# hustvl/InfiniteVL

Measured on AMD Instinct MI355X. Metric: prefill tok/s + decode tok/s, InfiniteVL-3B @128K seq, higher is better.
Workload: dtype bf16; 1 GPU; InfiniteVL-3B (36 layers: 9 SWA + 27 Gated DeltaNet, random-init bf16) streaming prefill, 256-token hipGraph chunk steps, SWA window 4096 (full); global_batch=1, seq_len=150016, parallelism=dp1 (batch-sharded replicas, one logits all-gather)

## Files before the change

### include/ivl_hip.h

```cpp
#ifndef IVL_HIP_H
#define IVL_HIP_H

#include <stddef.h>
#include <stdint.h>

#ifdef __cplusplus
extern "C" {
#endif

#define IVL_ABI_VERSION 11

#define IVL_API __attribute__((visibility("default")))

#define IVL_BF16 0
#define IVL_F32 2
#define IVL_FP8_E4M3 3

#define IVL_OK 0
#define IVL_ERR_INVALID_ARG (-1)
#define IVL_ERR_UNSUPPORTED (-2)
#define IVL_ERR_WORKSPACE (-3)
#define IVL_ERR_LAUNCH (-4)
#define IVL_ERR_SYNC (-5)

IVL_API int ivl_abi_version(void);
IVL_API const char* ivl_last_error(void);

IVL_API int ivl_gdn_recurrent_fwd(const void* q, const void* k, const void* v, const float* g, const void* beta,
                          void* o, const void* h0, int h0_dtype, void* ht, int ht_dtype,
                          int B, int T, int H, int K, int V, float scale, int use_qk_l2norm, void* stream);
IVL_API int ivl_gdn_recurrent_f16_fwd(const void* q, const void* k, const void* v, const float* g, const void* beta,
                              void* o, const void* h0, int h0_dtype, void* ht, int ht_dtype,
                              int B, int T, int H, int K, int V, float scale, int use_qk_l2norm, void* stream);

IVL_API size_t ivl_gdn_chunk_workspace_bytes(int B, int T, int H, int K, int V);
IVL_API int ivl_gdn_chunk_fwd(const void* q, const void* k, const void* v, const float* g, const void* beta,
                      void* o, const void* h0, int h0_dtype, void* ht, int ht_dtype,
                      int B, int T, int H, int K, int V, float scale, int use_qk_l2norm, int mma_dtype,
                      void* workspace, size_t workspace_bytes, void* stream);

#define IVL_GDN_SYNC_BYTES 16384
IVL_API int ivl_gdn_chunk_fused_fwd(const void* proj, int64_t ld, int col_q, int col_k, int col_v, int col_a, int col_b,
                            const void* wq, const void* wk, const void* wv, const void* sq_in, const void* sk_in,
                            const void* sv_in, void* sq_out, void* sk_out, void* sv_out, const float* A_log,
                            const float* dt_bias, void* o, const void* h0, int h0_dtype, void* ht, int ht_dtype, int B,
                            int T, int H, int K, int V, int conv_width, float scale, int mma_dtype, void* workspace,
                            size_t workspace_bytes, void* sync, void* stream);
IVL_API int ivl_gdn_sync_status(const void* sync, void* stream);
IVL_API int ivl_gdn_sync_reset(void* sync, void* stream);
#define IVL_GDN_RESIDENT_QUERY (-2147483647 - 1)
IVL_API int ivl_gdn_resident_blocks(int override_blocks);

IVL_API int ivl_gdn_gate_fwd(const void* a, const void* b, const float* A_log, const float* dt_bias,
                     float* g, void* beta, int rows, int H, void* stream);

IVL_API int ivl_short_conv_fwd(const void* x, const void* weight, const void* state_in, void* y, void* state_out,
                       int B, int T, int D, int W, int apply_silu, void* stream);
IVL_API int ivl_short_conv_bias_fwd(const void* x, const void* weight, const void* bias, const void* state_in, void* y, void* state_out,
                            int B, int T, int D, int W, int apply_silu, void* stream);

IVL_API int ivl_rmsnorm_swish_gate_fwd(const void* x, const void* gate, const void* weight, void* y,
                               int rows, int N, float eps, void* stream);
IVL_API int ivl_rmsnorm_swish_gate_res_fwd(const void* x, const void* gate, const void* weight, const void* residual, int residual_dtype,
                                   void* residual_out, int residual_out_dtype, void* y, int rows, int N, float eps, void* stream);

IVL_API int ivl_mrope_fwd(void* q, void* k, const void* cos, const void* sin,
                  int B, int T, int Hq, int Hkv, int d, int s0, int s1, int s2, void* stream);

typedef struct ivl_swa_args {
  const void* q;
  const void* k_new;
  const void* v_new;
  const void* k_cache;
  const void* v_cache;
  void* o;
  int64_t q_sb, q_st, q_sh;
  int64_t kn_sb, kn_st, kn_sh;
  int B, T, T_new, Hq, Hkv, d;
  int cache_capacity;
  int window;
  int64_t pos;
  const int64_t* pos_dev;
  float scaling;
  void* workspace;
  size_t workspace_bytes;
  const void* rope_cos;
  const void* rope_sin;
  int rope_s0, rope_s1;
  int mma_dtype;
  int append_new;
  int64_t pos_min;
} ivl_swa_args;

IVL_API size_t ivl_swa_workspace_bytes(int B, int T, int Hq, int d);
IVL_API size_t ivl_swa_ring256_workspace_bytes(int B, int T, int Hq, int Hkv, int d, int cache_capacity);
IVL_API int ivl_swa_fwd(const ivl_swa_args* args, void* stream);
IVL_API int ivl_swa_decode_rows_fwd(const ivl_swa_args* args, const int64_t* pos_rows, void* stream);

IVL_API int ivl_swa_cache_append(const void* k_new, const void* v_new, int64_t kn_sb, int64_t kn_st, int64_t kn_sh,
                         void* k_cache, void* v_cache, int B, int T, int Hkv, int d, int cache_capacity,
                         int64_t pos, const int64_t* pos_dev, const void* rope_cos, const void* rope_sin,
                         int rope_s0, int rope_s1, void* stream);

IVL_API int ivl_rope_tables_fwd(const int64_t* position_ids, const float* inv_freq, void* cos_out, void* sin_out, int rows,
                        int half_dim, float attention_scaling, void* stream);

IVL_API size_t ivl_vision_attn_workspace_bytes(int S, int H, int d, int max_seqlen);
IVL_API int ivl_vision_attn_fwd(const void* q, const void* k, const void* v, void* o,
                        int64_t q_st, int64_t q_sh, int64_t k_st, int64_t k_sh, int64_t v_st, int64_t v_sh,
                        int64_t o_st, int64_t o_sh, const int32_t* cu_seqlens, int n_seg, int max_seqlen,
                        int S, int H, int d, float scaling, const float* rope_cos, const float* rope_sin,
                        void* workspace, size_t workspace_bytes, void* stream);

IVL_API int ivl_counter_add(int64_t* counter, int64_t delta, void* stream);


IVL_API int ivl_gdn_prologue_fwd(const void* proj, int64_t ld, int col_q, int col_k, int col_v, int col_a, int col_b,
                         const void* w_q, const void* w_k, const void* w_v,
                         const void* sq_in, const void* sk_in, const void* sv_in,
                         void* sq_out, void* sk_out, void* sv_out,
                         const float* A_log, const float* dt_bias,
                         void* q, void* k, void* v, float* g, void* beta,
                         int B, int T, int H, int Dq, int Dk, int Dv, int W, int apply_silu, void* stream);

IVL_API int ivl_rmsnorm_swish_gate_strided_fwd(const void* x, const void* gate, int64_t gate_ld, int H,
                                       const void* weight, void* y, int rows, int N, float eps, void* stream);

IVL_API int ivl_mrope_strided_fwd(void* q, void* k, int64_t q_ld, int64_t k_ld, const void* cos, const void* sin,
                          int B, int T, int Hq, int Hkv, int d, int s0, int s1, int s2, void* stream);

IVL_API int ivl_add_rmsnorm_fwd(const void* x, const void* residual, const void* weight, void* y, void* h_out,
                        int rows, int N, float eps, void* stream);

IVL_API int ivl_silu_mul_fwd(const void* gate_up, void* y, int64_t rows, int I, void* stream);

IVL_API int ivl_gdn_decode_step_fwd(const void* proj, int64_t ld, int col_q, int col_k, int col_v, int col_g, int col_a,
                            int col_b, const void* conv_wq, const void* conv_wk, const void* conv_wv,
                            void* conv_state_q, void* conv_state_k, void* conv_state_v, const float* A_log,
                            const float* dt_bias, const void* norm_weight, float eps, void* state, int state_dtype,
                            void* y, int B, int H, int K, int V, float scale, void* stream);

IVL_API int ivl_gdn_decode_split_fwd(const void* proj, int64_t ld, int col_q, int col_k, int col_v, int col_a, int col_b,
                             const void* conv_wq, const void* conv_wk, const void* conv_wv, const void* conv_state_q,
                             const void* conv_state_k, void* conv_state_v, const float* A_log, const float* dt_bias,
                             void* state, int state_dtype, void* o_raw, int B, int H, int K, int V, float scale, void* stream);
IVL_API int ivl_gdn_out_linear_small_m_fwd(const void* o_raw, const void* gate, int64_t gate_ld, const void* norm_weight, float eps,
                                   int H, const void* proj, int64_t proj_ld, int col_q, int col_k, void* conv_state_q,
                                   void* conv_state_k, const void* w, const void* bias, void* y, int M, int N, int K, void* stream);

IVL_API int ivl_linear_small_m_fwd(const void* x, const void* w, const void* bias, void* y, int M, int N, int K, void* stream);

IVL_API int ivl_linear_swiglu_small_m_fwd(const void* x, const void* w_gate_up, const void* bias, void* y, int M, int I, int K,
                                  void* stream);

IVL_API int ivl_norm_linear_small_m_fwd(const void* x, const void* residual, const void* norm_weight, float eps, void* h_out,
                                const void* w, const void* bias, void* y, int M, int N, int K, int glu, void* stream);

#ifdef __cplusplus
}
#endif
#endif
```

### infinitevl_amd/_lib.py

```python
from __future__ import annotations

import ctypes
import os
from ctypes import POINTER, Structure, c_char_p, c_float, c_int, c_int64, c_size_t, c_void_p

_HERE = os.path.dirname(os.path.abspath(__file__))
LIB_PATH = os.path.join(_HERE, "libivl_hip.so")

IVL_BF16, IVL_F32, IVL_FP8_E4M3 = 0, 2, 3
IVL_OK = 0
IVL_GDN_SYNC_BYTES = 16384
IVL_GDN_RESIDENT_QUERY = -2147483648
IVL_ERR_INVALID_ARG, IVL_ERR_UNSUPPORTED, IVL_ERR_WORKSPACE, IVL_ERR_LAUNCH, IVL_ERR_SYNC = -1, -2, -3, -4, -5

EXPORTED_SYMBOLS = (
    "ivl_abi_version", "ivl_last_error",
    "ivl_gdn_recurrent_fwd", "ivl_gdn_chunk_workspace_bytes", "ivl_gdn_chunk_fwd", "ivl_gdn_gate_fwd",
    "ivl_short_conv_fwd", "ivl_rmsnorm_swish_gate_fwd", "ivl_mrope_fwd",
    "ivl_swa_workspace_bytes", "ivl_swa_fwd", "ivl_swa_cache_append", "ivl_counter_add",
    "ivl_gdn_prologue_fwd", "ivl_rmsnorm_swish_gate_strided_fwd", "ivl_mrope_strided_fwd",
    "ivl_add_rmsnorm_fwd", "ivl_silu_mul_fwd", "ivl_linear_small_m_fwd",
    "ivl_linear_swiglu_small_m_fwd", "ivl_gdn_decode_step_fwd", "ivl_gdn_chunk_fused_fwd", "ivl_rope_tables_fwd",
    "ivl_vision_attn_workspace_bytes", "ivl_vision_attn_fwd", "ivl_norm_linear_small_m_fwd",
    "ivl_gdn_sync_status", "ivl_gdn_sync_reset", "ivl_gdn_resident_blocks",
    "ivl_short_conv_bias_fwd", "ivl_rmsnorm_swish_gate_res_fwd", "ivl_gdn_recurrent_f16_fwd",
    "ivl_gdn_decode_split_fwd", "ivl_gdn_out_linear_small_m_fwd", "ivl_swa_ring256_workspace_bytes",
    "ivl_swa_decode_rows_fwd",
)


class SwaArgs(Structure):
    _fields_ = [
        ("q", c_void_p), ("k_new", c_void_p), ("v_new", c_void_p), ("k_cache", c_void_p), ("v_cache", c_void_p),
        ("o", c_void_p),
        ("q_sb", c_int64), ("q_st", c_int64), ("q_sh", c_int64),
        ("kn_sb", c_int64), ("kn_st", c_int64), ("kn_sh", c_int64),
        ("B", c_int), ("T", c_int), ("T_new", c_int), ("Hq", c_int), ("Hkv", c_int), ("d", c_int),
        ("cache_capacity", c_int), ("window", c_int),
        ("pos", c_int64), ("pos_dev", c_void_p),
        ("scaling", c_float),
        ("workspace", c_void_p), ("workspace_bytes", c_size_t),
        ("rope_cos", c_void_p), ("rope_sin", c_void_p), ("rope_s0", c_int), ("rope_s1", c_int),
        ("mma_dtype", c_int), ("append_new", c_int),
        ("pos_min", c_int64),
    ]


class IvlError(RuntimeError):
    def __init__(self, code: int, msg: str):
        super().__init__(f"libivl_hip error {code}: {msg}")
        self.code = code


_lib = None


def load(path: str = None) -> ctypes.CDLL:
    global _lib
    if _lib is not None:
        return _lib
    if path is not None:
        globals()["LIB_PATH"] = path
    if not os.path.exists(LIB_PATH):
        raise ImportError(
            f"{LIB_PATH} not found. The MI355X kernels are mandatory (there is no CPU or PyTorch fallback): "
            "build them with `python -c 'import __graft_entry__ as g; g.build()'` or `make -C infinitevl_amd/csrc`.")
    lib = ctypes.CDLL(LIB_PATH)
    vp, i, f, sz, i64 = c_void_p, c_int, c_float, c_size_t, c_int64
    lib.ivl_abi_version.restype = i
    lib.ivl_abi_version.argtypes = []
    lib.ivl_last_error.restype = c_char_p
    lib.ivl_last_error.argtypes = []
    lib.ivl_gdn_recurrent_fwd.restype = i
    lib.ivl_gdn_recurrent_fwd.argtypes = [vp, vp, vp, vp, vp, vp, vp, i, vp, i, i, i, i, i, i, f, i, vp]
    lib.ivl_gdn_chunk_workspace_bytes.restype = sz
    lib.ivl_gdn_chunk_workspace_bytes.argtypes = [i, i, i, i, i]
    lib.ivl_gdn_chunk_fwd.restype = i
    lib.ivl_gdn_chunk_fwd.argtypes = [vp, vp, vp, vp, vp, vp, vp, i, vp, i, i, i, i, i, i, f, i, i, vp, sz, vp]
    lib.ivl_gdn_chunk_fused_fwd.restype = i
    lib.ivl_gdn_chunk_fused_fwd.argtypes = ([vp, c_int64, i, i, i, i, i] + [vp] * 9 + [vp, vp, vp, vp, i, vp, i] +
                                            [i, i, i, i, i, i, f, i, vp, sz, vp, vp])
    if path is None or hasattr(lib, "ivl_gdn_sync_status"):
        lib.ivl_gdn_sync_status.restype = i
        lib.ivl_gdn_sync_status.argtypes = [vp, vp]
        lib.ivl_gdn_sync_reset.restype = i
        lib.ivl_gdn_sync_reset.argtypes = [vp, vp]
        lib.ivl_gdn_resident_blocks.restype = i
        lib.ivl_gdn_resident_blocks.argtypes = [i]
        lib.ivl_short_conv_bias_fwd.restype = i
        lib.ivl_short_conv_bias_fwd.argtypes = [vp, vp, vp, vp, vp, vp, i, i, i, i, i, vp]
        lib.ivl_rmsnorm_swish_gate_res_fwd.restype = i
        lib.ivl_rmsnorm_swish_gate_res_fwd.argtypes = [vp, vp, vp, vp, i, vp, i, vp, i, i, f, vp]
        lib.ivl_gdn_recurrent_f16_fwd.restype = i
        lib.ivl_gdn_recurrent_f16_fwd.argtypes = [vp, vp, vp, vp, vp, vp, vp, i, vp, i, i, i, i, i, i, f, i, vp]
    lib.ivl_rope_tables_fwd.restype = i
    lib.ivl_rope_tables_fwd.argtypes = [vp, vp, vp, vp, i, i, f, vp]
    lib.ivl_vision_attn_workspace_bytes.restype = sz
    lib.ivl_vision_attn_workspace_bytes.argtypes = [i, i, i, i]
    lib.ivl_vision_attn_fwd.restype = i
    lib.ivl_vision_attn_fwd.argtypes = [vp, vp, vp, vp] + [c_int64] * 8 + [vp, i, i, i, i, i, f, vp, vp, vp, sz, vp]
    lib.ivl_gdn_gate_fwd.restype = i
    lib.ivl_gdn_gate_fwd.argtypes = [vp, vp, vp, vp, vp, vp, i, i, vp]
    lib.ivl_short_conv_fwd.restype = i
    lib.ivl_short_conv_fwd.argtypes = [vp, vp, vp, vp, vp, i, i, i, i, i, vp]
    lib.ivl_rmsnorm_swish_gate_fwd.restype = i
    lib.ivl_rmsnorm_swish_gate_fwd.argtypes = [vp, vp, vp, vp, i, i, f, vp]
    lib.ivl_mrope_fwd.restype = i
    lib.ivl_mrope_fwd.argtypes = [vp, vp, vp, vp, i, i, i, i, i, i, i, i, vp]
    lib.ivl_swa_workspace_bytes.restype = sz
    lib.ivl_swa_workspace_bytes.argtypes = [i, i, i, i]
    lib.ivl_swa_ring256_workspace_bytes.restype = sz
    lib.ivl_swa_ring256_workspace_bytes.argtypes = [i, i, i, i, i, i]
    lib.ivl_swa_fwd.restype = i
    lib.ivl_swa_fwd.argtypes = [POINTER(SwaArgs), vp]
    if path is None or hasattr(lib, "ivl_swa_decode_rows_fwd"):
        lib.ivl_swa_decode_rows_fwd.restype = i
        lib.ivl_swa_decode_rows_fwd.argtypes = [POINTER(SwaArgs), vp, vp]
    lib.ivl_swa_cache_append.restype = i
    lib.ivl_swa_cache_append.argtypes = [vp, vp, i64, i64, i64, vp, vp, i, i, i, i, i, i64, vp, vp, vp, i, i, vp]
    lib.ivl_counter_add.restype = i
    lib.ivl_counter_add.argtypes = [vp, i64, vp]
    lib.ivl_gdn_prologue_fwd.restype = i
    lib.ivl_gdn_prologue_fwd.argtypes = [vp, i64, i, i, i, i, i, vp, vp, vp, vp, vp, vp, vp, vp, vp, vp, vp,
                                         vp, vp, vp, vp, vp, i, i, i, i, i, i, i, i, vp]
    lib.ivl_rmsnorm_swish_gate_strided_fwd.restype = i
    lib.ivl_rmsnorm_swish_gate_strided_fwd.argtypes = [vp, vp, i64, i, vp, vp, i, i, f, vp]
    lib.ivl_mrope_strided_fwd.restype = i
    lib.ivl_mrope_strided_fwd.argtypes = [vp, vp, i64, i64, vp, vp, i, i, i, i, i, i, i, i, vp]
    lib.ivl_add_rmsnorm_fwd.restype = i
    lib.ivl_add_rmsnorm_fwd.argtypes = [vp, vp, vp, vp, vp, i, i, f, vp]
    lib.ivl_silu_mul_fwd.restype = i
    lib.ivl_silu_mul_fwd.argtypes = [vp, vp, i64, i, vp]
    lib.ivl_linear_small_m_fwd.restype = i
    lib.ivl_linear_small_m_fwd.argtypes = [vp, vp, vp, vp, i, i, i, vp]
    lib.ivl_gdn_decode_step_fwd.restype = i
    lib.ivl_gdn_decode_step_fwd.argtypes = [vp, i64, i, i, i, i, i, i, vp, vp, vp, vp, vp, vp, vp, vp, vp, f, vp, i,
                                            vp, i, i, i, i, f, vp]
    if path is None or hasattr(lib, "ivl_gdn_decode_split_fwd"):
        lib.ivl_gdn_decode_split_fwd.restype = i
        lib.ivl_gdn_decode_split_fwd.argtypes = [vp, i64, i, i, i, i, i, vp, vp, vp, vp, vp, vp, vp, vp, vp, i, vp, i, i, i, i, f, vp]
        lib.ivl_gdn_out_linear_small_m_fwd.restype = i
        lib.ivl_gdn_out_linear_small_m_fwd.argtypes = [vp, vp, i64, vp, f, i, vp, i64, i, i, vp, vp, vp, vp, vp, i, i, i, vp]
    lib.ivl_linear_swiglu_small_m_fwd.restype = i
    lib.ivl_linear_swiglu_small_m_fwd.argtypes = [vp, vp, vp, vp, i, i, i, vp]
    lib.ivl_norm_linear_small_m_fwd.restype = i
    lib.ivl_norm_linear_small_m_fwd.argtypes = [vp, vp, vp, f, vp, vp, vp, vp, i, i, i, i, vp]
    _lib = lib
    env = os.environ.get("IVL_GDN_RESIDENT_BLOCKS", "")
    if env.strip() and hasattr(lib, "ivl_gdn_resident_blocks"):
        lib.ivl_gdn_resident_blocks(int(env))
    return lib


def check(rc: int) -> None:
    if rc == IVL_OK:
        return
    msg = load().ivl_last_error().decode("utf-8", "replace")
    if rc in (IVL_ERR_INVALID_ARG, IVL_ERR_UNSUPPORTED):
        raise ValueError(f"libivl_hip ({rc}): {msg}")
    raise IvlError(rc, msg)
```

### infinitevl_amd/ops.py

```python
from __future__ import annotations

import contextlib
import ctypes
import os
import threading
import weakref
from typing import Dict, Optional, Tuple

import torch
import torch.nn as nn

from . import _lib
from ._lib import IVL_BF16, IVL_F32, IVL_FP8_E4M3, SwaArgs

_DT_CODE = {torch.bfloat16: IVL_BF16, torch.float32: IVL_F32}
_MMA_CODE = {None: IVL_BF16, "bf16": IVL_BF16, torch.bfloat16: IVL_BF16, "fp8": IVL_FP8_E4M3, "fp8_e4m3": IVL_FP8_E4M3,
             getattr(torch, "float8_e4m3fn", "fp8_e4m3"): IVL_FP8_E4M3}


def mma_code(mma_dtype) -> int:
    try:
        return _MMA_CODE[mma_dtype]
    except KeyError:
        raise ValueError(f"mma_dtype must be None, 'bf16' or 'fp8_e4m3' (got {mma_dtype!r})") from None
# ... 439 lines not shown
        return self.hidden_size * self.kernel_size[0]

    def forward(self, x: torch.Tensor, mask: Optional[torch.Tensor] = None, cache: Optional[torch.Tensor] = None,
                output_final_state: bool = False, cu_seqlens: Optional[torch.Tensor] = None, **kwargs):
        _need_gpu(x)
        if cu_seqlens is not None:
            if x.shape[0] != 1:
                raise ValueError(f"The batch size is expected to be 1 rather than {x.shape[0]} when using `cu_seqlens`.")
            if mask is not None:
                raise ValueError("`mask` and `cu_seqlens` cannot be provided at the same time")
            segs = _varlen_segments(cu_seqlens, x.shape[1])
            if x.dtype != torch.bfloat16:
                raise ValueError(f"ShortConvolution kernel is built for bf16, got {x.dtype}")
            x = x.contiguous()
            D, W = x.shape[2], self.kernel_size[0]
            if cache is not None and (cache.dtype != torch.bfloat16 or not cache.is_contiguous()
                                      or tuple(cache.shape) != (len(segs), D, W)):
                raise ValueError(f"conv cache must be a contiguous bf16 [N,D,W] = {(len(segs), D, W)} tensor (one row block per "
                                 f"sequence of cu_seqlens); got {cache.dtype} {tuple(cache.shape)}")
            state_in = cache
            if cache is None and output_final_state:
                cache = torch.zeros(len(segs), D, W, dtype=x.dtype, device=x.device)
            y = torch.empty_like(x)
            for i, (a, b_) in enumerate(segs):
                if b_ > a:
                    self._launch(x[:, a:b_], y[:, a:b_], None if state_in is None else state_in[i:i + 1],
                                 None if cache is None else cache[i:i + 1], 1, b_ - a, D, W)
            return y, cache
        if mask is not None:
            x = x.mul(mask.unsqueeze(-1))
        if x.dtype != torch.bfloat16:
            raise ValueError(f"ShortConvolution kernel is built for bf16, got {x.dtype}")
        B, T, D = x.shape
        W = self.kernel_size[0]
        x = x.contiguous()
        state_in = cache
        if output_final_state and cache is None:
            cache = torch.empty(B, D, W, dtype=x.dtype, device=x.device)
        if cache is not None and (cache.dtype != torch.bfloat16 or not cache.is_contiguous()
                                  or tuple(cache.shape) != (B, D, W)):
            raise ValueError("conv cache must be a contiguous bf16 [N,D,W] tensor")
        y = torch.empty_like(x)
        self._launch(x, y, state_in, cache, B, T, D, W)
        return y, cache

    def _launch(self, x, y, state_in, state_out, B, T, D, W) -> None:
        w = self.weight
        if w.dtype != torch.bfloat16:
            w = w.to(torch.bfloat16)
        if self.bias is not None:
            _lib.check(_lib.load().ivl_short_conv_bias_fwd(
                _p(x), _p(w.contiguous()), _p(self.bias.to(torch.bfloat16).contiguous()), _p(state_in), _p(y), _p(state_out), B, T, D, W,
                int(self.activation is not None), _stream(x)))
        else:
            _lib.check(_lib.load().ivl_short_conv_fwd(
                _p(x), _p(w.contiguous()), _p(state_in), _p(y), _p(state_out), B, T, D, W,
                int(self.activation is not None), _stream(x)))

    def step(self, x: torch.Tensor, cache: torch.Tensor):
        return self.forward(x, cache=cache, output_final_state=True)


class FusedRMSNormGated(nn.Module):

    def __init__(self, hidden_size: int, elementwise_affine: bool = True, eps: float = 1e-5,
                 activation: str = "swish", device=None, dtype=None):
        super().__init__()
        if activation not in ("swish", "silu"):
            raise ValueError(f"Unsupported activation: {activation}")
        self.hidden_size, self.elementwise_affine, self.eps, self.activation = hidden_size, elementwise_affine, eps, activation
        if elementwise_affine:
            self.weight = nn.Parameter(torch.ones(hidden_size, device=device, dtype=dtype))
        else:
            self.register_parameter("weight", None)
        self.register_parameter("bias", None)

    def forward(self, x: torch.Tensor, g: torch.Tensor, residual=None, prenorm=False, residual_in_fp32=False):
        _need_gpu(x, g, residual)
        if x.dtype != torch.bfloat16:
            raise ValueError(f"FusedRMSNormGated kernel is built for bf16, got {x.dtype}")
        N = x.shape[-1]
        x, g = x.contiguous(), g.contiguous()
        y = torch.empty_like(x)
        if self.weight is None:
            w = torch.ones(N, dtype=torch.bfloat16, device=x.device)
        else:
            w = self.weight if self.weight.dtype == torch.bfloat16 else self.weight.to(torch.bfloat16)
        if residual is not None or prenorm or residual_in_fp32:
            if residual is not None:
                if residual.dtype not in _DT_CODE or tuple(residual.shape) != tuple(x.shape):
                    raise ValueError("residual must be a bf16 / fp32 tensor of x's shape")
                residual = residual.contiguous()
            res_dt = residual.dtype if residual is not None else (torch.float32 if residual_in_fp32 else None)
            res_out = torch.empty(x.shape, dtype=res_dt, device=x.device) if res_dt is not None and (residual is not None or res_dt != x.dtype) else None
            _lib.check(_lib.load().ivl_rmsnorm_swish_gate_res_fwd(
                _p(x), _p(g), _p(w.contiguous()), _p(residual), _DT_CODE[residual.dtype] if residual is not None else IVL_BF16,
                _p(res_out), _DT_CODE[res_out.dtype] if res_out is not None else IVL_BF16, _p(y), x.numel() // N, N, float(self.eps), _stream(x)))
            return y if not prenorm else (y, res_out if res_out is not None else x)
        _lib.check(_lib.load().ivl_rmsnorm_swish_gate_fwd(_p(x), _p(g), _p(w.contiguous()), _p(y),
                                                          x.numel() // N, N, float(self.eps), _stream(x)))
        return y


class RMSNorm(nn.Module):

    def __init__(self, hidden_size: int, elementwise_affine: bool = True, bias: bool = False, eps: float = 1e-5,
                 device=None, dtype=None):
        super().__init__()
        if bias:
            raise NotImplementedError("InfiniteVL's norms carry no bias")
        self.hidden_size, self.elementwise_affine, self.eps = hidden_size, elementwise_affine, eps
        self.register_parameter("weight", None)
        self.register_parameter("bias", None)
        if elementwise_affine:
            self.weight = nn.Parameter(torch.ones(hidden_size, device=device, dtype=dtype))

    def extra_repr(self) -> str:
        return f"{self.hidden_size}, eps={self.eps}" + ("" if self.elementwise_affine else ", elementwise_affine=False")

    def forward(self, x: torch.Tensor, residual=None, prenorm: bool = False, residual_in_fp32: bool = False):
        if residual is not None or prenorm:
            raise NotImplementedError("residual/prenorm are not used by InfiniteVL (std:1341)")
        w = self.weight if self.weight is not None else torch.ones(self.hidden_size, dtype=x.dtype, device=x.device)
        if self.hidden_size == 256 and x.dtype == torch.bfloat16:
            _need_gpu(x)
            xc = x.contiguous()
            y = torch.empty_like(xc)
            _lib.check(_lib.load().ivl_rmsnorm_swish_gate_fwd(_p(xc), None, _p(w.to(torch.bfloat16).contiguous()), _p(y),
                                                              xc.numel() // 256, 256, float(self.eps), _stream(xc)))
            return y
        y, _ = add_rmsnorm(x, None, w, self.eps)
        return y


def get_unpad_data(attention_mask: torch.Tensor):
    lens = attention_mask.sum(dim=-1, dtype=torch.int32)
    indices = torch.nonzero(attention_mask.flatten(), as_tuple=False).flatten()
    cu = torch.nn.functional.pad(torch.cumsum(lens, dim=0, dtype=torch.int32), (1, 0))
    return indices, cu, int(lens.max().item()) if lens.numel() else 0


def index_first_axis(x: torch.Tensor, indices: torch.Tensor) -> torch.Tensor:
    return x.index_select(0, indices)


def pad_input(x: torch.Tensor, indices: torch.Tensor, batch: int, seqlen: int) -> torch.Tensor:
    out = torch.zeros(batch * seqlen, *x.shape[1:], dtype=x.dtype, device=x.device)
    out.index_copy_(0, indices, x)
    return out.view(batch, seqlen, *x.shape[1:])


def gdn_prologue(proj: torch.Tensor, cols, conv_weights, conv_states_in, conv_states_out, A_log32, dt_bias32,
                 H: int, Dq: int, Dk: int, Dv: int):
    _need_gpu(proj)
    B, T, ld = proj.shape
    assert proj.is_contiguous() and proj.dtype == torch.bfloat16
    dev = proj.device
    q = torch.empty(B, T, Dq, dtype=torch.bfloat16, device=dev)
    k = torch.empty(B, T, Dk, dtype=torch.bfloat16, device=dev)
    v = torch.empty(B, T, Dv, dtype=torch.bfloat16, device=dev)
    g = torch.empty(B, T, H, dtype=torch.float32, device=dev)
    beta = torch.empty(B, T, H, dtype=torch.bfloat16, device=dev)
    wq, wk, wv = conv_weights
    si, so = conv_states_in, conv_states_out
    _lib.check(_lib.load().ivl_gdn_prologue_fwd(
        _p(proj), ld, cols[0], cols[1], cols[2], cols[3], cols[4], _p(wq), _p(wk), _p(wv),
        _p(si[0]), _p(si[1]), _p(si[2]), _p(so[0]), _p(so[1]), _p(so[2]), _p(A_log32), _p(dt_bias32),
        _p(q), _p(k), _p(v), _p(g), _p(beta), B, T, H, Dq, Dk, Dv, wq.shape[-1], 1, _stream(proj)))
    return q, k, v, g, beta


def gdn_decode_step(proj: torch.Tensor, cols, conv_weights, conv_states, A_log32, dt_bias32, norm_weight, eps: float,
                    state: torch.Tensor, H: int, K: int, V: int, scale: float) -> torch.Tensor:
    _need_gpu(proj, state)
    B, T, ld = proj.shape
    assert T == 1 and proj.is_contiguous() and proj.dtype == torch.bfloat16 and state.is_contiguous()
    y = torch.empty(B, 1, H * V, dtype=torch.bfloat16, device=proj.device)
    wq, wk, wv = conv_weights
    sq, sk, sv = conv_states
    _lib.check(_lib.load().ivl_gdn_decode_step_fwd(
        _p(proj), ld, cols[0], cols[1], cols[2], cols[3], cols[4], cols[5], _p(wq), _p(wk), _p(wv), _p(sq), _p(sk), _p(sv),
        _p(A_log32), _p(dt_bias32), _p(norm_weight), float(eps), _p(state), _DT_CODE[state.dtype], _p(y), B, H, K, V,
        float(scale), _stream(proj)))
    return y


_SPLIT_DECODE = False


def gdn_decode_split(proj: torch.Tensor, cols, conv_weights, conv_states, A_log32, dt_bias32, state: torch.Tensor,
                     H: int, K: int, V: int, scale: float) -> torch.Tensor:
    _need_gpu(proj, state)
    B, T, ld = proj.shape
    assert T == 1 and proj.is_contiguous() and proj.dtype == torch.bfloat16 and state.is_contiguous()
    o_raw = torch.empty(B, 1, H * V, dtype=torch.bfloat16, device=proj.device)
    wq, wk, wv = conv_weights
    sq, sk, sv = conv_states
    _lib.check(_lib.load().ivl_gdn_decode_split_fwd(
        _p(proj), ld, cols[0], cols[1], cols[2], cols[3], cols[4], _p(wq), _p(wk), _p(wv), _p(sq), _p(sk), _p(sv),
        _p(A_log32), _p(dt_bias32), _p(state), _DT_CODE[state.dtype], _p(o_raw), B, H, K, V, float(scale), _stream(proj)))
    return o_raw


def gdn_out_linear(o_raw: torch.Tensor, proj: torch.Tensor, col_g: int, col_q: int, col_k: int, norm_weight: torch.Tensor, eps: float,
                   conv_state_q: torch.Tensor, conv_state_k: torch.Tensor, weight: torch.Tensor, bias: Optional[torch.Tensor],
                   H: int) -> torch.Tensor:
    _need_gpu(o_raw, proj, weight)
    B, T, ld = proj.shape
    K = o_raw.shape[-1]
    N = weight.shape[0]
    assert T == 1 and o_raw.is_contiguous() and weight.is_contiguous() and weight.dtype == torch.bfloat16
    y = torch.empty(B, 1, N, dtype=torch.bfloat16, device=o_raw.device)
    gate = proj.view(B, ld)[:, col_g:]
    _lib.check(_lib.load().ivl_gdn_out_linear_small_m_fwd(
        _p(o_raw), ctypes.c_void_p(gate.data_ptr()), ld, _p(norm_weight), float(eps), H, _p(proj), ld, col_q, col_k,
        _p(conv_state_q), _p(conv_state_k), _p(weight), _p(bias) if bias is not None else None, _p(y), B, N, K, _stream(o_raw)))
    return y


def rmsnorm_swish_gate_strided(x: torch.Tensor, gate_base: torch.Tensor, gate_ld: int, weight: torch.Tensor,
                               eps: float) -> torch.Tensor:
    _need_gpu(x, gate_base)
    B, T, H, N = x.shape
    y = torch.empty_like(x)
    _lib.check(_lib.load().ivl_rmsnorm_swish_gate_strided_fwd(_p(x), _p(gate_base), gate_ld, H, _p(weight), _p(y),
                                                              B * T * H, N, float(eps), _stream(x)))
    return y


def add_rmsnorm(x: torch.Tensor, residual: Optional[torch.Tensor], weight: torch.Tensor, eps: float):
    _need_gpu(x, residual)
    if x.dtype != torch.bfloat16:
        raise ValueError("add_rmsnorm is built for bf16")
    N = x.shape[-1]
    x = x.contiguous()
    y = torch.empty_like(x)
    h = torch.empty_like(x) if residual is not None else None
    w = weight if weight.dtype == torch.bfloat16 else weight.to(torch.bfloat16)
    _lib.check(_lib.load().ivl_add_rmsnorm_fwd(_p(x), _p(residual.contiguous()) if residual is not None else None,
                                               _p(w), _p(y), _p(h), x.numel() // N, N, float(eps), _stream(x)))
    return y, (h if h is not None else x)


_PRENORM = True


class PreNorm:

    def __init__(self, x: torch.Tensor, residual: Optional[torch.Tensor], weight: torch.Tensor, eps: float):
        self.x = x if x.is_contiguous() else x.contiguous()
        self.residual = None if residual is None else (residual if residual.is_contiguous() else residual.contiguous())
        self.weight = weight if weight.dtype == torch.bfloat16 else weight.to(torch.bfloat16)
        self.eps = float(eps)
        self.h = torch.empty_like(self.x) if residual is not None else self.x
        self.shape, self.dtype, self.device, self.is_cuda = self.x.shape, self.x.dtype, self.x.device, self.x.is_cuda
        self._y = None
        self.done = False

    def size(self, *a):
        return self.x.size(*a)

    def dim(self):
        return self.x.dim()

    def numel(self):
        return self.x.numel()

    def materialize(self) -> torch.Tensor:
        if self._y is None:
            N = self.x.shape[-1]
            self._y = torch.empty_like(self.x)
            _lib.check(_lib.load().ivl_add_rmsnorm_fwd(_p(self.x), _p(self.residual), _p(self.weight), _p(self._y),
                                                       _p(self.h) if self.residual is not None else None,
                                                       self.x.numel() // N, N, self.eps, _stream(self.x)))
            self.done = True
        return self._y


def _prenorm_linear(pn: "PreNorm", weight: torch.Tensor, bias: Optional[torch.Tensor], glu: bool) -> Optional[torch.Tensor]:
    K = weight.shape[-1]
    rows = pn.numel() // K if K else 0
    if not (pn.is_cuda and 1 <= rows <= 4 and pn.dtype == torch.bfloat16 and weight.dtype == torch.bfloat16 and weight.dim() == 2
            and weight.is_contiguous() and K % 8 == 0 and 512 <= K <= 4096 and pn.shape[-1] == K and pn._y is None
            and (bias is None or (bias.dtype == torch.bfloat16 and bias.is_contiguous()))):
        return None
    N = weight.shape[0] // 2 if glu else weight.shape[0]
    y = torch.empty(*pn.shape[:-1], N, dtype=torch.bfloat16, device=pn.device)
    _lib.check(_lib.load().ivl_norm_linear_small_m_fwd(
        _p(pn.x), _p(pn.residual), _p(pn.weight), pn.eps, _p(pn.h) if pn.residual is not None else None,
        _p(weight), _p(bias) if bias is not None else None, _p(y), rows, N, K, 1 if glu else 0, _stream(pn.x)))
    pn.done = True
    return y


def silu_mul(gate_up: torch.Tensor) -> torch.Tensor:
    _need_gpu(gate_up)
    assert gate_up.is_contiguous() and gate_up.dtype == torch.bfloat16
    I = gate_up.shape[-1] // 2
    y = torch.empty(*gate_up.shape[:-1], I, dtype=torch.bfloat16, device=gate_up.device)
    _lib.check(_lib.load().ivl_silu_mul_fwd(_p(gate_up), _p(y), gate_up.numel() // (2 * I), I, _stream(gate_up)))
    return y


def linear(x: torch.Tensor, weight: torch.Tensor, bias: Optional[torch.Tensor] = None) -> torch.Tensor:
    if isinstance(x, PreNorm):
        y = _prenorm_linear(x, weight, bias, False)
        if y is not None:
            return y
        x = x.materialize()
    K = weight.shape[-1]
    rows = x.numel() // K if K else 0
    if (x.is_cuda and 1 <= rows <= 4 and x.dtype == torch.bfloat16 and weight.dtype == torch.bfloat16
            and weight.dim() == 2 and weight.is_contiguous() and K % 8 == 0
            and (bias is None or (bias.dtype == torch.bfloat16 and bias.is_contiguous()))):
        xc = x if x.is_contiguous() else x.contiguous()
        N = weight.shape[0]
        y = torch.empty(*x.shape[:-1], N, dtype=torch.bfloat16, device=x.device)
        _lib.check(_lib.load().ivl_linear_small_m_fwd(_p(xc), _p(weight), _p(bias) if bias is not None else None,
                                                      _p(y), rows, N, K, _stream(x)))
        return y
    return torch.nn.functional.linear(x, weight, bias)


def linear_swiglu(x: torch.Tensor, w_gate_up: torch.Tensor) -> torch.Tensor:
    if isinstance(x, PreNorm):
        y = _prenorm_linear(x, w_gate_up, None, True)
        if y is not None:
            return y
        x = x.materialize()
    K = w_gate_up.shape[-1]
    I = w_gate_up.shape[0] // 2
    rows = x.numel() // K
    if (x.is_cuda and 1 <= rows <= 4 and x.dtype == torch.bfloat16 and w_gate_up.dtype == torch.bfloat16
            and w_gate_up.is_contiguous() and K % 8 == 0):
        xc = x if x.is_contiguous() else x.contiguous()
        y = torch.empty(*x.shape[:-1], I, dtype=torch.bfloat16, device=x.device)
        _lib.check(_lib.load().ivl_linear_swiglu_small_m_fwd(_p(xc), _p(w_gate_up), None, _p(y), rows, I, K, _stream(x)))
        return y
    return silu_mul(linear(x, w_gate_up))


def apply_mrope_strided_inplace(q: torch.Tensor, k: torch.Tensor, cos: torch.Tensor, sin: torch.Tensor, mrope_section):
    _need_gpu(q, k, cos, sin)
    B, T, Hq, d = q.shape
    Hkv = k.shape[2]
    assert q.stride(3) == 1 and q.stride(2) == d and k.stride(3) == 1 and k.stride(2) == d

    def row_stride(t_):
        if T > 1 and B > 1:
            assert t_.stride(0) == T * t_.stride(1), "q/k must be row-uniform views of a [B*T, ld] buffer"
        return t_.stride(1) if T > 1 else t_.stride(0)
    cos = cos.to(torch.bfloat16).contiguous()
    sin = sin.to(torch.bfloat16).contiguous()
    s0, s1, s2 = (int(s) for s in mrope_section)
    _lib.check(_lib.load().ivl_mrope_strided_fwd(_p(q), _p(k), row_stride(q), row_stride(k), _p(cos), _p(sin),
                                                 B, T, Hq, Hkv, d, s0, s1, s2, _stream(q)))
    return q, k


def apply_mrope_inplace(q: torch.Tensor, k: torch.Tensor, cos: torch.Tensor, sin: torch.Tensor, mrope_section):
    _need_gpu(q, k, cos, sin)
    B, T, Hq, d = q.shape
    Hkv = k.shape[2]
    assert q.is_contiguous() and k.is_contiguous() and q.dtype == k.dtype == torch.bfloat16
    cos = cos.to(torch.bfloat16).contiguous()
    sin = sin.to(torch.bfloat16).contiguous()
    if cos.shape[0] != 3 or tuple(cos.shape[1:]) != (B, T, d):
        raise ValueError(f"cos/sin must be [3,B,T,d]; got {tuple(cos.shape)}")
    s0, s1, s2 = (int(s) for s in mrope_section)
    _lib.check(_lib.load().ivl_mrope_fwd(_p(q), _p(k), _p(cos), _p(sin), B, T, Hq, Hkv, d, s0, s1, s2, _stream(q)))
    return q, k


SWA_RING256 = os.environ.get("IVL_SWA_RING256", "1") != "0"
SWA_RING256_CALLS = 0


def swa_forward(
    q: torch.Tensor, k_new: torch.Tensor, v_new: torch.Tensor, *, window: Optional[int], scaling: float,
    k_cache: Optional[torch.Tensor] = None, v_cache: Optional[torch.Tensor] = None,
    pos: int = 0, pos_dev: Optional[torch.Tensor] = None, n_query: Optional[int] = None,
    layout: str = "bthd", mma_dtype=None, rope=None, append: bool = False, pos_min: int = 0, pos_min_holds_in_graph: bool = False,
    pos_rows: Optional[torch.Tensor] = None,
) -> torch.Tensor:
    _need_gpu(q, k_new, v_new, k_cache, v_cache, pos_dev, pos_rows)
    if q.dtype != torch.bfloat16 or k_new.dtype != torch.bfloat16 or v_new.dtype != torch.bfloat16:
        raise ValueError("swa_forward is built for bf16")
    if layout == "bhtd":
        q, k_new, v_new = q.transpose(1, 2), k_new.transpose(1, 2), v_new.transpose(1, 2)
    B, T, Hq, d = q.shape
    T_new, Hkv = k_new.shape[1], k_new.shape[2]
    if n_query is not None:
        assert n_query == T
    if pos_rows is not None:
        if pos_dev is not None or pos != 0 or pos_min != 0:
            raise ValueError("swa_forward: pos_rows excludes pos / pos_dev / pos_min")
        if pos_rows.dtype != torch.int64 or tuple(pos_rows.shape) != (B,) or not pos_rows.is_contiguous():
            raise ValueError(f"swa_forward: pos_rows must be a contiguous int64 [B] = [{B}] tensor; got {pos_rows.dtype} "
                             f"{tuple(pos_rows.shape)}")
        if k_cache is None:
            raise ValueError("swa_forward: pos_rows needs a ring cache (k_cache / v_cache)")
        if T_new != T or T * (Hq // Hkv) > 64:
            raise ValueError(f"swa_forward: pos_rows serves packed decode steps only: T_new == T and T * Hq/Hkv <= 64 "
                             f"(got T={T}, T_new={T_new}, Hq/Hkv={Hq // Hkv})")
        if mma_code(mma_dtype) != IVL_BF16:
            raise ValueError("swa_forward: pos_rows runs in bf16 only (no fp8 decode step)")
    if q.stride(-1) != 1:
        q = q.contiguous()
    if k_new.stride(-1) != 1 or v_new.stride() != k_new.stride():
        k_new, v_new = k_new.contiguous(), v_new.contiguous()
    C = 0
    if k_cache is not None:
        assert k_cache.is_contiguous() and v_cache.is_contiguous() and k_cache.dtype == torch.bfloat16
        assert tuple(k_cache.shape[:2]) == (B, Hkv) and k_cache.shape[3] == d
        C = k_cache.shape[2]
    o = torch.empty(B, T, Hq, d, dtype=torch.bfloat16, device=q.device)
    lib = _lib.load()
    nbytes = lib.ivl_swa_workspace_bytes(B, T, Hq, d)
    pos_min = int(pos_min) if pos_dev is not None else int(pos)
    if pos_rows is not None or not (SWA_RING256 and C > 0 and pos_min >= C and T >= 256 and T_new == T and window == C + 1) or (
            torch.cuda.is_current_stream_capturing() and not pos_min_holds_in_graph):
        pos_min = 0
    else:
        n256 = lib.ivl_swa_ring256_workspace_bytes(B, T, Hq, Hkv, d, C)
        if n256 > 0 and mma_code(mma_dtype) == IVL_BF16:
            global SWA_RING256_CALLS
            SWA_RING256_CALLS += 1
        nbytes = max(nbytes, n256)
    ws = get_workspace(nbytes, q.device, "swa")
    a = SwaArgs()
    a.q, a.k_new, a.v_new, a.k_cache, a.v_cache, a.o = (q.data_ptr(), k_new.data_ptr(), v_new.data_ptr(),
                                                         k_cache.data_ptr() if C else None,
                                                         v_cache.data_ptr() if C else None, o.data_ptr())
    a.q_sb, a.q_st, a.q_sh = q.stride(0), q.stride(1), q.stride(2)
    a.kn_sb, a.kn_st, a.kn_sh = k_new.stride(0), k_new.stride(1), k_new.stride(2)
    a.B, a.T, a.T_new, a.Hq, a.Hkv, a.d = B, T, T_new, Hq, Hkv, d
    a.cache_capacity = C
    a.window = int(window) if window is not None else 0
    a.pos = int(pos)
    a.pos_dev = pos_dev.data_ptr() if pos_dev is not None else None
    a.scaling = float(scaling)
    a.workspace, a.workspace_bytes = ws.data_ptr(), ws.numel()
    a.mma_dtype = mma_code(mma_dtype)
    a.append_new = int(bool(append) and C > 0)
    a.pos_min = pos_min
    if rope is not None:
        cos, sin, sec = _rope_args(rope, B, T, d)
        a.rope_cos, a.rope_sin, a.rope_s0, a.rope_s1 = cos.data_ptr(), sin.data_ptr(), int(sec[0]), int(sec[1])
    if pos_rows is not None:
        _lib.check(lib.ivl_swa_decode_rows_fwd(ctypes.byref(a), pos_rows.data_ptr(), _stream(q)))
    else:
        _lib.check(lib.ivl_swa_fwd(ctypes.byref(a), _stream(q)))
    return o


def _rope_args(rope, B: int, T: int, d: int):
    cos, sin, sec = rope
    if cos.dtype != torch.bfloat16 or not cos.is_contiguous():
        cos = cos.to(torch.bfloat16).contiguous()
    if sin.dtype != torch.bfloat16 or not sin.is_contiguous():
        sin = sin.to(torch.bfloat16).contiguous()
    if tuple(cos.shape) != (3, B, T, d) or tuple(sin.shape) != (3, B, T, d):
        raise ValueError(f"rope cos/sin must be [3,B,T,d] = {(3, B, T, d)}; got {tuple(cos.shape)}")
    return cos, sin, sec


def swa_cache_append(k_new: torch.Tensor, v_new: torch.Tensor, k_cache: torch.Tensor, v_cache: torch.Tensor,
                     pos: int = 0, pos_dev: Optional[torch.Tensor] = None, rope=None) -> None:
    _need_gpu(k_new, v_new, k_cache, v_cache)
    B, T, Hkv, d = k_new.shape
    if k_new.stride(-1) != 1 or v_new.stride() != k_new.stride():
        k_new, v_new = k_new.contiguous(), v_new.contiguous()
    rc = rs = None
    s0 = s1 = 0
    if rope is not None:
        rc, rs, sec = _rope_args(rope, B, T, d)
        s0, s1 = int(sec[0]), int(sec[1])
    _lib.check(_lib.load().ivl_swa_cache_append(
        _p(k_new), _p(v_new), k_new.stride(0), k_new.stride(1), k_new.stride(2), _p(k_cache), _p(v_cache),
        B, T, Hkv, d, k_cache.shape[2], int(pos), _p(pos_dev), _p(rc), _p(rs), s0, s1, _stream(k_new)))


def counter_add(counter: torch.Tensor, delta: int) -> None:
    _lib.check(_lib.load().ivl_counter_add(_p(counter), int(delta), _stream(counter)))


def swa_attention_interface(module, query, key, value, attention_mask=None, dropout: float = 0.0,
                            scaling: Optional[float] = None, sliding_window: Optional[int] = None,
                            position_ids=None, **kwargs):
    if dropout:
        raise NotImplementedError("attention dropout is a training feature; the hot path is inference")
    if scaling is None:
        scaling = query.shape[-1] ** -0.5
    out = swa_forward(query, key, value, window=sliding_window, scaling=scaling, layout="bhtd")
    return out, None
```

Before: 48640 tok/s.

## Add fused 256-row SwiGLU GEMM kernel for prefill chunk MLP

Adds a custom HIP MFMA GEMM specialised for exactly 256 rows that loads x and weight tiles straight into LDS through a 3-stage ring and applies bias plus SiLU-gate times up in the epilogue. In the MLP of the 256-token chunk steps it replaces the hipBLAS linear followed by a separate silu_mul kernel, which removes the round trip of the 2I-wide intermediate through memory. Weight loads use non-temporal hints. The trade-off is that a hand-written kernel may reach lower GEMM throughput than the vendor library.

```diff
diff --git a/include/ivl_hip.h b/include/ivl_hip.h
--- a/include/ivl_hip.h
+++ b/include/ivl_hip.h
@@ -156,6 +156,8 @@
 IVL_API int ivl_norm_linear_small_m_fwd(const void* x, const void* residual, const void* norm_weight, float eps, void* h_out,
                                 const void* w, const void* bias, void* y, int M, int N, int K, int glu, void* stream);
 
+IVL_API int ivl_linear_m256_fwd(const void* x, const void* w, const void* bias, void* y, int M, int N, int K, int glu, void* stream);
+
 #ifdef __cplusplus
 }
 #endif
diff --git a/infinitevl_amd/_lib.py b/infinitevl_amd/_lib.py
--- a/infinitevl_amd/_lib.py
+++ b/infinitevl_amd/_lib.py
@@ -25,7 +25,7 @@
     "ivl_gdn_sync_status", "ivl_gdn_sync_reset", "ivl_gdn_resident_blocks",
     "ivl_short_conv_bias_fwd", "ivl_rmsnorm_swish_gate_res_fwd", "ivl_gdn_recurrent_f16_fwd",
     "ivl_gdn_decode_split_fwd", "ivl_gdn_out_linear_small_m_fwd", "ivl_swa_ring256_workspace_bytes",
-    "ivl_swa_decode_rows_fwd",
+    "ivl_swa_decode_rows_fwd", "ivl_linear_m256_fwd",
 )
 
 
@@ -145,6 +145,8 @@
     lib.ivl_linear_swiglu_small_m_fwd.argtypes = [vp, vp, vp, vp, i, i, i, vp]
     lib.ivl_norm_linear_small_m_fwd.restype = i
     lib.ivl_norm_linear_small_m_fwd.argtypes = [vp, vp, vp, f, vp, vp, vp, vp, i, i, i, i, vp]
+    lib.ivl_linear_m256_fwd.restype = i
+    lib.ivl_linear_m256_fwd.argtypes = [vp, vp, vp, vp, i, i, i, i, vp]
     _lib = lib
     env = os.environ.get("IVL_GDN_RESIDENT_BLOCKS", "")
     if env.strip() and hasattr(lib, "ivl_gdn_resident_blocks"):
diff --git a/infinitevl_amd/csrc/linear_m256.hip b/infinitevl_amd/csrc/linear_m256.hip
--- /dev/null
+++ b/infinitevl_amd/csrc/linear_m256.hip
@@ -0,0 +1,215 @@
+#include "ivl_common.h"
+
+namespace ivl {
+
+constexpr int L256_ROWS = 256;
+constexpr int L256_BK = 64;
+constexpr int L256_KMAX = 16384;
+#ifndef L256_WG_ROWS
+#define L256_WG_ROWS 256
+#endif
+#ifndef L256_STAGES
+#define L256_STAGES 3
+#endif
+#ifndef L256_W_NT
+#define L256_W_NT 1
+#endif
+
+template <bool GLU, int ROWS, int NST>
+struct L256Cfg {
+  static constexpr int NCOL = GLU ? 48 : 64;
+  static constexpr int NW = GLU ? 2 * NCOL : NCOL;
+  static constexpr int NT = NW / 16;
+  static constexpr int WAVES = ROWS / 32;
+  static constexpr int PIECES = (ROWS + NW) / 8;
+  static constexpr int PW_MAX = (PIECES + WAVES - 1) / WAVES;
+  static constexpr int STAGE = (ROWS + NW) * 128;
+  static constexpr int LDS = NST * STAGE;
+};
+
+template <int N>
+__device__ __forceinline__ void l256_vmcnt() {
+  static_assert(N >= 0 && N < 64, "vmcnt immediate");
+  asm volatile("s_waitcnt vmcnt(%0)" ::"n"(N) : "memory");
+}
+
+template <int PW>
+__device__ __forceinline__ void l256_wait_tiles(int ahead) {
+  if (ahead <= 0) l256_vmcnt<0>();
+  else if (ahead == 1) l256_vmcnt<PW>();
+  else l256_vmcnt<2 * PW>();
+}
+
+__device__ __forceinline__ const bf16_t* l256_uniform(const bf16_t* p) {
+  const unsigned long long v = (unsigned long long)p;
+  const unsigned int lo = __builtin_amdgcn_readfirstlane((unsigned int)v), hi = __builtin_amdgcn_readfirstlane((unsigned int)(v >> 32));
+  return (const bf16_t*)(((unsigned long long)hi << 32) | lo);
+}
+
+template <bool GLU, int ROWS, int NST, bool WNT>
+__global__ __launch_bounds__(ROWS * 2) void linear_m256_kernel(const bf16_t* __restrict__ x, const bf16_t* __restrict__ w,
+                                                               const bf16_t* __restrict__ bias, bf16_t* __restrict__ y, int M, int N, int K) {
+  using C = L256Cfg<GLU, ROWS, NST>;
+  static_assert(NST >= 2 && NST <= 3, "ring of 2 or 3 stages");
+  constexpr int AHEAD = NST - 1;
+  extern __shared__ __attribute__((aligned(16))) unsigned char smem[];
+  const int tid = threadIdx.x, lane = tid & 63, wave = __builtin_amdgcn_readfirstlane(tid >> 6);
+  int colblk = (int)blockIdx.x, r0 = 0;
+  if constexpr (ROWS < L256_ROWS) {
+    const int b = (int)blockIdx.x;
+    colblk = (b >> 4) * 8 + (b & 7);
+    r0 = ((b >> 3) & 1) * ROWS;
+    if (colblk * C::NCOL >= N || r0 >= M) return;
+  }
+  const int n0 = colblk * C::NCOL;
+  const int nkt = K / L256_BK;
+  const unsigned int lds_base = (unsigned int)(size_t)smem;
+
+  const bool pw_full = wave < C::PIECES % C::WAVES || C::PIECES % C::WAVES == 0;
+  unsigned int src_off[C::PW_MAX];
+#pragma unroll
+  for (int i = 0; i < C::PW_MAX; ++i) {
+    const int p = min(wave + C::WAVES * i, C::PIECES - 1);
+    const int r = 8 * p + (lane >> 3);
+    const int c = (lane & 7) ^ ((r >> 1) & 7);
+    long long grow;
+    if (r < ROWS) {
+      grow = min(r0 + r, M - 1);
+    } else {
+      const int j = r - ROWS;
+      if (GLU) grow = j < C::NCOL ? min(n0 + j, N - 1) : (long long)N + min(n0 + j - C::NCOL, N - 1);
+      else grow = min(n0 + j, N - 1);
+    }
+    src_off[i] = (unsigned int)(grow * K * 2 + c * 16);
+  }
+  auto dma_tile = [&](int t) __attribute__((always_inline)) {
+    const unsigned int dst0 = lds_base + (unsigned int)(t % NST) * C::STAGE;
+    const bf16_t* xb = l256_uniform(x + (size_t)t * L256_BK);
+    const bf16_t* wb = l256_uniform(w + (size_t)t * L256_BK);
+#pragma unroll
+    for (int i = 0; i < C::PW_MAX; ++i) {
+      const int p = wave + C::WAVES * i;
+      if (i == C::PW_MAX - 1 && p >= C::PIECES) break;
+      const unsigned int dst = __builtin_amdgcn_readfirstlane(dst0 + 1024u * p);
+      unsigned int keep;
+      if (p < ROWS / 8 || !WNT)
+        asm volatile("s_mov_b32 %0, m0\n\ts_mov_b32 m0, %2\n\ts_nop 0\n\tglobal_load_lds_dwordx4 %1, %3\n\ts_mov_b32 m0, %0"
+                     : "=&s"(keep) : "v"(src_off[i]), "s"(dst), "s"(p < ROWS / 8 ? xb : wb) : "memory");
+      else
+        asm volatile("s_mov_b32 %0, m0\n\ts_mov_b32 m0, %2\n\ts_nop 0\n\tglobal_load_lds_dwordx4 %1, %3 nt\n\ts_mov_b32 m0, %0"
+                     : "=&s"(keep) : "v"(src_off[i]), "s"(dst), "s"(wb) : "memory");
+    }
+  };
+
+  unsigned int frag_off[2];
+#pragma unroll
+  for (int s = 0; s < 2; ++s) frag_off[s] = (unsigned int)((lane & 15) * 128 + (((4 * s + (lane >> 4)) ^ ((lane >> 1) & 7)) << 4));
+
+  f32x4 acc[C::NT][2];
+#pragma unroll
+  for (int j = 0; j < C::NT; ++j)
+#pragma unroll
+    for (int i = 0; i < 2; ++i) acc[j][i] = f32x4{0.f, 0.f, 0.f, 0.f};
+
+#pragma unroll
+  for (int t = 0; t < AHEAD; ++t)
+    if (t < nkt) dma_tile(t);
+  for (int t = 0; t < nkt; ++t) {
+    const int ahead = min(AHEAD - 1, nkt - 1 - t);
+    if (pw_full) l256_wait_tiles<C::PW_MAX>(ahead);
+    else l256_wait_tiles<C::PW_MAX - 1>(ahead);
+    asm volatile("s_waitcnt lgkmcnt(0)\n\ts_barrier" ::: "memory");
+    if (t + AHEAD < nkt) dma_tile(t + AHEAD);
+    const unsigned char* st = smem + (t % NST) * C::STAGE;
+#pragma unroll
+    for (int s = 0; s < 2; ++s) {
+      bf16x8 xf[2], wf[C::NT];
+#pragma unroll
+      for (int i = 0; i < 2; ++i) xf[i] = *(const bf16x8*)(st + (32 * wave + 16 * i) * 128 + frag_off[s]);
+#pragma unroll
+      for (int j = 0; j < C::NT; ++j) wf[j] = *(const bf16x8*)(st + (ROWS + 16 * j) * 128 + frag_off[s]);
+#pragma unroll
+      for (int j = 0; j < C::NT; ++j)
+#pragma unroll
+        for (int i = 0; i < 2; ++i) acc[j][i] = __builtin_amdgcn_mfma_f32_16x16x32_bf16(wf[j], xf[i], acc[j][i], 0, 0, 0);
+    }
+  }
+
+  const int cq = 4 * (lane >> 4);
+  if constexpr (GLU) {
+#pragma unroll
+    for (int j = 0; j < C::NT / 2; ++j) {
+      const int col = n0 + 16 * j + cq;
+      float bg[4] = {0.f, 0.f, 0.f, 0.f}, bu[4] = {0.f, 0.f, 0.f, 0.f};
+      if (bias != nullptr && col < N)
+#pragma unroll
+        for (int r = 0; r < 4; ++r) { bg[r] = bf2f(bias[col + r]); bu[r] = bf2f(bias[N + col + r]); }
+#pragma unroll
+      for (int i = 0; i < 2; ++i) {
+        const int row = r0 + 32 * wave + 16 * i + (lane & 15);
+        float o[4];
+#pragma unroll
+        for (int r = 0; r < 4; ++r) {
+          const float g = bf_round(acc[j][i][r] + bg[r]), u = bf_round(acc[j + C::NT / 2][i][r] + bu[r]);
+          o[r] = bf_round(g * sigmoidf_(g)) * u;
+        }
+        if (row < M && col < N) store_out8(y + (size_t)row * N + col, u32x2{pack2bf(o[0], o[1]), pack2bf(o[2], o[3])});
+      }
+    }
+  } else {
+#pragma unroll
+    for (int j = 0; j < C::NT; ++j) {
+      const int col = n0 + 16 * j + cq;
+      float bb[4] = {0.f, 0.f, 0.f, 0.f};
+      if (bias != nullptr && col < N)
+#pragma unroll
+        for (int r = 0; r < 4; ++r) bb[r] = bf2f(bias[col + r]);
+#pragma unroll
+      for (int i = 0; i < 2; ++i) {
+        const int row = r0 + 32 * wave + 16 * i + (lane & 15);
+        if (row < M && col < N)
+          store_out8(y + (size_t)row * N + col,
+                     u32x2{pack2bf(acc[j][i][0] + bb[0], acc[j][i][1] + bb[1]), pack2bf(acc[j][i][2] + bb[2], acc[j][i][3] + bb[3])});
+      }
+    }
+  }
+}
+
+template <bool GLU>
+static int launch_l256(const void* x, const void* w, const void* bias, void* y, int M, int N, int K, hipStream_t st) {
+  constexpr int ROWS = L256_WG_ROWS, NST = L256_STAGES;
+  using C = L256Cfg<GLU, ROWS, NST>;
+  constexpr bool WNT = GLU && L256_W_NT != 0;
+  const void* fn = (const void*)linear_m256_kernel<GLU, ROWS, NST, WNT>;
+  static bool attr_set[64];
+  int dev = 0;
+  (void)hipGetDevice(&dev);
+  if (!__atomic_load_n(&attr_set[dev & 63], __ATOMIC_ACQUIRE)) {
+    (void)hipFuncSetAttribute(fn, hipFuncAttributeMaxDynamicSharedMemorySize, C::LDS);
+    __atomic_store_n(&attr_set[dev & 63], true, __ATOMIC_RELEASE);
+  }
+  const int ncol = (N + C::NCOL - 1) / C::NCOL;
+  const dim3 grid(ROWS < L256_ROWS ? (ncol + 7) / 8 * 16 : ncol);
+  hipLaunchKernelGGL((linear_m256_kernel<GLU, ROWS, NST, WNT>), grid, dim3(ROWS * 2), C::LDS, st, (const bf16_t*)x,
+                     (const bf16_t*)w, (const bf16_t*)bias, (bf16_t*)y, M, N, K);
+  return check_launch("ivl_linear_m256_fwd");
+}
+
+}
+
+using namespace ivl;
+
+extern "C" int ivl_linear_m256_fwd(const void* x, const void* w, const void* bias, void* y, int M, int N, int K, int glu, void* stream) {
+  IVL_REQUIRE(x && w && y, IVL_ERR_INVALID_ARG, "ivl_linear_m256_fwd: NULL pointer");
+  IVL_REQUIRE(M > 0 && N > 0 && K > 0, IVL_ERR_INVALID_ARG, "ivl_linear_m256_fwd: M=%d N=%d K=%d", M, N, K);
+  IVL_REQUIRE(M <= L256_ROWS, IVL_ERR_UNSUPPORTED, "ivl_linear_m256_fwd: M=%d (built for at most %d rows)", M, L256_ROWS);
+  IVL_REQUIRE(K % L256_BK == 0 && K <= L256_KMAX, IVL_ERR_UNSUPPORTED,
+              "ivl_linear_m256_fwd: K=%d (a multiple of %d, at most %d)", K, L256_BK, L256_KMAX);
+  IVL_REQUIRE(N % 4 == 0, IVL_ERR_UNSUPPORTED, "ivl_linear_m256_fwd: N=%d (a multiple of 4: 8-byte output pieces)", N);
+  IVL_REQUIRE((long long)(glu ? 2 : 1) * N * K * 2 < (1ll << 32), IVL_ERR_UNSUPPORTED,
+              "ivl_linear_m256_fwd: weight of %d x %d rows does not fit 32-bit offsets", glu ? 2 * N : N, K);
+  IVL_REQUIRE((((size_t)x | (size_t)w) & 15) == 0 && ((size_t)y & 7) == 0 && ((size_t)bias & 1) == 0, IVL_ERR_INVALID_ARG,
+              "ivl_linear_m256_fwd: x / w must be 16-byte aligned, y 8-byte aligned");
+  hipStream_t st = (hipStream_t)stream;
+  return glu ? launch_l256<true>(x, w, bias, y, M, N, K, st) : launch_l256<false>(x, w, bias, y, M, N, K, st);
+}
diff --git a/infinitevl_amd/ops.py b/infinitevl_amd/ops.py
--- a/infinitevl_amd/ops.py
+++ b/infinitevl_amd/ops.py
@@ -765,6 +765,19 @@
     return y
 
 
+def _m256_swiglu_applies(x: torch.Tensor, w_gate_up: torch.Tensor, rows: int, I: int, K: int) -> bool:
+    return (x.is_cuda and rows == 256 and 6144 < I <= 12288 and I % 4 == 0 and K % 64 == 0 and 64 <= K <= 16384
+            and x.dtype == torch.bfloat16 and w_gate_up.dtype == torch.bfloat16 and w_gate_up.dim() == 2
+            and w_gate_up.is_contiguous() and x.is_contiguous() and x.shape[-1] == K and x.data_ptr() % 16 == 0
+            and w_gate_up.data_ptr() % 16 == 0)
+
+
+def _linear_swiglu_m256(x: torch.Tensor, w_gate_up: torch.Tensor, rows: int, I: int, K: int) -> torch.Tensor:
+    y = torch.empty(*x.shape[:-1], I, dtype=torch.bfloat16, device=x.device)
+    _lib.check(_lib.load().ivl_linear_m256_fwd(_p(x), _p(w_gate_up), None, _p(y), rows, I, K, 1, _stream(x)))
+    return y
+
+
 def linear(x: torch.Tensor, weight: torch.Tensor, bias: Optional[torch.Tensor] = None) -> torch.Tensor:
     if isinstance(x, PreNorm):
         y = _prenorm_linear(x, weight, bias, False)
@@ -800,6 +813,8 @@
         y = torch.empty(*x.shape[:-1], I, dtype=torch.bfloat16, device=x.device)
         _lib.check(_lib.load().ivl_linear_swiglu_small_m_fwd(_p(xc), _p(w_gate_up), None, _p(y), rows, I, K, _stream(x)))
         return y
+    if _m256_swiglu_applies(x, w_gate_up, rows, I, K):
+        return _linear_swiglu_m256(x, w_gate_up, rows, I, K)
     return silu_mul(linear(x, w_gate_up))
 
 
```

After: 52090 tok/s, median of 6. 1.07x the previous value.
